# Antibas/eaQHM-analysis-and-synthesis-in-Python

Measured on AMD Instinct MI355X. Metric: analysis_frames_per_sec, higher is better.
Workload: dtype f64; 1 GPU; synth16k_60s_female_maxAdpt5; samples=960000, fs=16000, ls_frames_per_adaptation=63936, adaptations_executed=5, Kmax=59, track_bytes=906240000, parallelism=instants sharded x1 by LS cost; boundary records all-gathered per adaptation

## Files before the change

### eaqhm-analysis-and-synthesis-in-python_amd/csrc/eaqhm_ls_tile.hip

```cpp
#include <type_traits>
#include "eaqhm_ls_common.h"
#include "eaqhm_ls_chol.h"
#include "eaqhm_ls_a0.h"
#include "eaqhm_ls_tilemap.h"
#include "eaqhm_ls_twunits.h"

namespace eaqhm {


#define DIAG_OWNER(jb, nt) ((int)TL_DIAG[nt][jb])
#define TL_THREADS 512
#define TL_WAVES 8
#define TL_CW 8
#define TL_NTMAX 13
#define CI_STRIDE 20
#define CI_NCH 16
#define A0_NS 7
#define A0_M 7

#define TZ_TB 104
#define TZ_NCH 8

__device__ inline void tw_step(d4 (&g)[9], double aR, double aI, double bR, double bI, double nk) {
  const double sA = aR + aI, dB = bI - bR;
  const double naR = nk * aR, naI = nk * aI, nsA = nk * sA;
  const double nbR = nk * bR, nbI = nk * bI, ndB = nk * dB;
  g[0] = __builtin_amdgcn_mfma_f64_16x16x4f64(aR, bR, g[0], 0, 0, 0);
  g[1] = __builtin_amdgcn_mfma_f64_16x16x4f64(aI, bI, g[1], 0, 0, 0);
  g[2] = __builtin_amdgcn_mfma_f64_16x16x4f64(sA, dB, g[2], 0, 0, 0);
  g[3] = __builtin_amdgcn_mfma_f64_16x16x4f64(naR, bR, g[3], 0, 0, 0);
  g[4] = __builtin_amdgcn_mfma_f64_16x16x4f64(naI, bI, g[4], 0, 0, 0);
  g[5] = __builtin_amdgcn_mfma_f64_16x16x4f64(nsA, dB, g[5], 0, 0, 0);
  g[6] = __builtin_amdgcn_mfma_f64_16x16x4f64(naR, nbR, g[6], 0, 0, 0);
  g[7] = __builtin_amdgcn_mfma_f64_16x16x4f64(naI, nbI, g[7], 0, 0, 0);
  g[8] = __builtin_amdgcn_mfma_f64_16x16x4f64(nsA, ndB, g[8], 0, 0, 0);
}

__device__ inline void twu_pair_k3(d4 (&g0)[3], d4 (&g1)[3], d4 (&g2)[3], double aR, double aI, double bR, double bI, double nk) {
  const double sA = aR + aI, dB = bI - bR;
  const double naR = nk * aR, naI = nk * aI, nsA = nk * sA;
  const double nbR = nk * bR, nbI = nk * bI, ndB = nk * dB;
  g0[0] = __builtin_amdgcn_mfma_f64_16x16x4f64(aR, bR, g0[0], 0, 0, 0);
  g0[1] = __builtin_amdgcn_mfma_f64_16x16x4f64(aI, bI, g0[1], 0, 0, 0);
  g0[2] = __builtin_amdgcn_mfma_f64_16x16x4f64(sA, dB, g0[2], 0, 0, 0);
  g1[0] = __builtin_amdgcn_mfma_f64_16x16x4f64(naR, bR, g1[0], 0, 0, 0);
  g1[1] = __builtin_amdgcn_mfma_f64_16x16x4f64(naI, bI, g1[1], 0, 0, 0);
  g1[2] = __builtin_amdgcn_mfma_f64_16x16x4f64(nsA, dB, g1[2], 0, 0, 0);
  g2[0] = __builtin_amdgcn_mfma_f64_16x16x4f64(naR, nbR, g2[0], 0, 0, 0);
  g2[1] = __builtin_amdgcn_mfma_f64_16x16x4f64(naI, nbI, g2[1], 0, 0, 0);
  g2[2] = __builtin_amdgcn_mfma_f64_16x16x4f64(nsA, ndB, g2[2], 0, 0, 0);
}
__device__ inline void twu_pair_2acc(d4 (&g0)[2], d4 (&g1)[2], d4 (&g2)[2], double aR, double aI, double bR, double bI, double nk,
                                     bool k4) {
  const double naR = nk * aR, naI = nk * aI, nbR = nk * bR, nbI = nk * bI;
  g0[0] = __builtin_amdgcn_mfma_f64_16x16x4f64(aR, bR, g0[0], 0, 0, 0);
  g1[0] = __builtin_amdgcn_mfma_f64_16x16x4f64(naR, bR, g1[0], 0, 0, 0);
  g2[0] = __builtin_amdgcn_mfma_f64_16x16x4f64(naR, nbR, g2[0], 0, 0, 0);
  g0[1] = __builtin_amdgcn_mfma_f64_16x16x4f64(aR, bI, g0[1], 0, 0, 0);
  g1[1] = __builtin_amdgcn_mfma_f64_16x16x4f64(naR, bI, g1[1], 0, 0, 0);
  g2[1] = __builtin_amdgcn_mfma_f64_16x16x4f64(naR, nbI, g2[1], 0, 0, 0);
  g0[0] = __builtin_amdgcn_mfma_f64_16x16x4f64(aI, bI, g0[0], 0, 0, 0);
  g1[0] = __builtin_amdgcn_mfma_f64_16x16x4f64(naI, bI, g1[0], 0, 0, 0);
  g2[0] = __builtin_amdgcn_mfma_f64_16x16x4f64(naI, nbI, g2[0], 0, 0, 0);
  if (k4) {
    const double maI = -aI, mnaI = -naI;
    g0[1] = __builtin_amdgcn_mfma_f64_16x16x4f64(maI, bR, g0[1], 0, 0, 0);
    g1[1] = __builtin_amdgcn_mfma_f64_16x16x4f64(mnaI, bR, g1[1], 0, 0, 0);
    g2[1] = __builtin_amdgcn_mfma_f64_16x16x4f64(mnaI, nbR, g2[1], 0, 0, 0);
  }
}

template <int NS, int TW, int UA = 0, int UB = 0>
__device__ __attribute__((noinline)) void tile_frame(const LsArgs& A, int TS_, int ldx_max_, double* lds, int f_) {
  const int TS = uni(TS_), ldx_max = uni(ldx_max_), f = uni(f_);
  const int tid = threadIdx.x, nt_thr = TL_THREADS;
  const int lane = tid & 63;
  const int wave = __builtin_amdgcn_readfirstlane(tid >> 6);
  double* U = uni(lds);
  double* Xre = U;
  double* Xim = Xre + (size_t)TS * ldx_max;
  const size_t usize_g = (size_t)2 * TS * ldx_max;
  double* ci = U + usize_g;
  unsigned long long* masks = (unsigned long long*)(ci + (size_t)CI_STRIDE * 52);
  double* PanR = U;
  double* PanI = PanR + TL_NTMAX * TL_TILE;
  double* WtR = PanI + TL_NTMAX * TL_TILE;
  double* WtI = WtR + TL_NTMAX * TL_TILE;
  double* LdR = WtI + TL_NTMAX * TL_TILE;
  double* LdI = LdR + TL_TILE;
  double* Dc = LdI + TL_TILE;
  double* Zc = Dc + DG_TILE;
  double* zv = Zc + DG_TILE;
  double* xv = zv + 2 * 16 * TL_NTMAX;
  const size_t usize_c = (size_t)(xv + 32 - U);
  double* xs = U + usize_c;
  double* sh = xs + 4 * uni(A.Kcmax);
  double* win = sh + 16;
  double* sig = win + 64 * CI_NCH;
  double* dorig = sig + 64 * CI_NCH;

  const int Npad = ((uni(A.Nmax) + 63) >> 6) << 6;
  double* Qs = uni(A.scratch) + (size_t)blockIdx.x * (size_t)uni((int)A.scratch_stride);
  double* Rs = Qs + (size_t)Npad * uni(A.nmax);
  const bool seeds = uni((int)(A.any_seed && (*A.any_seed != 0))) != 0;
  const double w1 = uni(2.0 * M_PI / A.fs);
  const int PE = TS / 2;
  const double* sA = uni(A.s);
  const int lcol = lane & 15, lq = lane >> 4;
  unsigned long long* dbg = uni(A.debug);
  unsigned long long t_prev = 0;

  {
    const int n = uni(A.ncol[f]);
    const int Kc = 2 * n + 1, Ms = 2 * Kc + 1;
    const int nt = (Ms + 15) >> 4;
    const int c = uni(A.frame_c[f]), wl = uni(A.frame_wl[f]), inst = uni(A.frame_inst[f]);
    const int N = 2 * wl + 1, mid = wl;
    const int T = (Kc + 16) >> 4;
    constexpr int UN = UA + UB;
    constexpr int GA = UA / 3, GB = UB / 3;
    constexpr bool G3 = TW > 0 || UN > 0;
    static_assert(TW == 0 || UN == 0, "whole pairs or units");
    static_assert(UN == 0 || (UA == TWU_UA && UB == TWU_UB), "slot layout of eaqhm_ls_twunits.h");
    const int nb = G3 ? T : nt;
    const int ldx = (nb << 4) + ((nb & 1) ? 0 : 16);
    const int npair = T * (T + 1) / 2;
    const int is = 2 * Kc - 16 * (nt - 1);
    const double f0 = uni(A.f0_stale);
    const int* mycols = uni(A.cols) + (size_t)f * uni(A.Kmax);
    const int npairs = mid + 1;

    if (dbg && tid == 0) t_prev = __builtin_amdgcn_s_memtime();
    for (int q = tid; q < 2 * TS * ldx_max; q += nt_thr) Xre[q] = 0.0;
    for (int t = tid; t < N; t += nt_thr) {
      win[t] = window_value(false, t, N);
      sig[t] = sA[(size_t)(c - wl) + t];
    }
    __syncthreads();
    int* gappy = (int*)(masks + (size_t)52 * CI_NCH);
    prepare_slots<CI_STRIDE, TL_WAVES>(A, Qs, Rs, Npad, ci, masks, gappy, mycols, n, N, mid, c, wl, seeds, lane, wave, CI_NCH);
    LS_STAMP(0);

    constexpr int NM3 = (NS <= 7) ? NS : 0;
    d4 accR[NS], accI[NS], acc3[NM3 ? NM3 : 1];
    int tP[NS], tQ[NS];
    bool live[NS];
#pragma unroll
    for (int sl = 0; sl < NS; ++sl) {
      accR[sl] = (d4){0, 0, 0, 0};
      accI[sl] = (d4){0, 0, 0, 0};
      if (sl < NM3) acc3[sl] = (d4){0, 0, 0, 0};
      const int code = TL_MAP[nt][wave][sl];
      live[sl] = code != 0xFF;
      const int P = live[sl] ? (code >> 4) : 0, Q = live[sl] ? (code & 15) : 0;
      tP[sl] = __builtin_amdgcn_readfirstlane(P);
      tQ[sl] = __builtin_amdgcn_readfirstlane(Q);
    }

    constexpr int TWA = TW ? TW : 1;
    d4 g[TWA][9];
    int gI[TWA], gJ[TWA];
    bool glive[TWA];
#pragma unroll
    for (int sl = 0; sl < TWA; ++sl) {
      const int x = wave + 8 * sl;
      glive[sl] = TW && x < npair;
      int I = 0, J = 0;
      if (glive[sl]) tile_of(x, I, J);
      gI[sl] = __builtin_amdgcn_readfirstlane(I);
      gJ[sl] = __builtin_amdgcn_readfirstlane(J);
#pragma unroll
      for (int p = 0; p < 9; ++p) g[sl][p] = (d4){0, 0, 0, 0};
    }

    constexpr int UAA = UA > 3 ? UA : 3, UBA = UB > 3 ? UB : 3;
    d4 ga[UAA][3], gb[UBA][2];
    int ucode[UN ? UN : 1];
    if constexpr (UN > 0) {
#pragma unroll
      for (int sl = 0; sl < UN; ++sl) ucode[sl] = __builtin_amdgcn_readfirstlane((int)TWU_MAP[wave][sl]);
#pragma unroll
      for (int sl = 0; sl < UA; ++sl)
#pragma unroll
        for (int p = 0; p < 3; ++p) ga[sl][p] = (d4){0, 0, 0, 0};
#pragma unroll
      for (int sl = 0; sl < UB; ++sl) gb[sl][0] = gb[sl][1] = (d4){0, 0, 0, 0};
    }

    for (int d0 = 0; d0 < npairs; d0 += PE) {
#pragma clang loop unroll(disable)
      for (int idx = tid; idx < 16 * n; idx += nt_thr) {
        const int el = idx & 15, j = idx >> 4, d = d0 + el;
        const bool act = d <= mid;
        const int u = mid - d - 1, v = mid + d;
        double su = 0, cu = 1, sv, cv;
        double pur = 0, pui = 0, nur = 0, nui = 0, pvr, pvi, nvr, nvi;
        {
          double* cj = ci + j * CI_STRIDE;
          const double* fb = ((const double**)cj)[2];
          const double* ab = ((const double**)cj)[3];
          const int dc = act ? d : mid;
          const double fu1 = fb[mid - dc], fv = fb[mid + dc];
          const double au = ab[(mid - dc - 1 >= 0) ? (mid - dc - 1) : 0], au1 = ab[mid - dc];
          const double av = ab[mid + dc], av1 = ab[(mid + dc + 1 < N) ? (mid + dc + 1) : (N - 1)];
          const double xu = act ? fu1 : 0.0, xv = (act && d >= 1) ? fv : 0.0;
          const double qv = cj[0] + scan16(xv), qu = -(cj[1] + scan16(xu));
          if (el == 15) { cj[0] = qv; cj[1] = -qu; }
          if (!act) continue;
          const double ainv = cj[17], pr = cj[18], pi = cj[19];
          sincos_cw(qu * w1, &su, &cu);
          sincos_cw(qv * w1, &sv, &cv);
          const double eps = 10e-5;
          if (u >= 0) {
            const double ru = (eps + au) * ainv, rv1 = (eps + av1) * ainv;
            pur = ru * cu;                    pui = ru * su;
            nur = rv1 * (cv * pr - sv * pi);  nui = rv1 * (cv * pi + sv * pr);
          }
          const double rv = (eps + av) * ainv, ru1 = (eps + au1) * ainv;
          pvr = rv * cv;                      pvi = rv * sv;
          nvr = ru1 * (cu * pr - su * pi);    nvi = ru1 * (cu * pi + su * pr);
        }
        double* xr = Xre + (2 * el) * ldx;
        double* xi = Xim + (2 * el) * ldx;
        const int cpos = XCOL(n + 1 + j, el), cneg = XCOL(j, el);
        const int spos = XCOL(Kc + n + 1 + j, el), sneg = XCOL(Kc + j, el);
        const double wv = win[v], nv = (double)(v - mid);
        if (u >= 0) {
          const double wu = win[u], nu = (double)(u - mid);
          pur *= wu; pui *= wu; nur *= wu; nui *= wu;
          xr[cpos] = pur;      xi[cpos] = pui;      xr[cneg] = nur;      xi[cneg] = nui;
          if (!G3) { xr[spos] = nu * pur; xi[spos] = nu * pui; xr[sneg] = nu * nur; xi[sneg] = nu * nui; }
        }
        pvr *= wv; pvi *= wv; nvr *= wv; nvi *= wv;
        xr += ldx; xi += ldx;
        xr[cpos] = pvr;      xi[cpos] = pvi;      xr[cneg] = nvr;      xi[cneg] = nvi;
        if (!G3) { xr[spos] = nv * pvr; xi[spos] = nv * pvi; xr[sneg] = nv * nvr; xi[sneg] = nv * nvi; }
      }
      if ((tid & 15) == 0 && (tid >> 4) < TS) {
        const int row = tid >> 4;
        const int d = d0 + (row >> 1);
        const int t = (row & 1) ? (mid + d) : (mid - d - 1);
        const bool ok = (d <= mid) && (t >= 0);
        const double w = ok ? win[t] : 0.0;
        const double sval = ok ? sig[t] : 0.0;
        const double nn = (double)(t - mid);
        const int el = row >> 1;
        double* xr = Xre + row * ldx;
        double* xi = Xim + row * ldx;
        xr[XCOL(n, el)] = w;               xi[XCOL(n, el)] = 0.0;
        if (!G3) {
          xr[XCOL(Kc + n, el)] = w * nn;   xi[XCOL(Kc + n, el)] = 0.0;
        }
        const int scol = G3 ? Kc : 2 * Kc;
        xr[XCOL(scol, el)] = w * sval;     xi[XCOL(scol, el)] = 0.0;
      }
      if (d0 + PE > mid) {
        for (int q = tid; q < TS * 16 * nb; q += nt_thr) {
          const int row = q / (16 * nb), col = q - row * (16 * nb);
          const int d = d0 + (row >> 1);
          const int t = (row & 1) ? (mid + d) : (mid - d - 1);
          if (d > mid || t < 0) { Xre[row * ldx + col] = 0.0; Xim[row * ldx + col] = 0.0; }
        }
      }
      LS_STAMP(12);
      __syncthreads();
      LS_STAMP(1);
      const int pcs = (npairs - d0 < PE) ? (npairs - d0) : PE;
      const int ksl = (pcs + 1) >> 1;
      if constexpr (UN > 0) {
        const int plane = TS * ldx_max;
        const int kn = (ksl < 8) ? ksl : 8;
#pragma unroll
        for (int gi = 0; gi < GA + GB; ++gi) {
          const int s0 = (gi < GA) ? 3 * gi : UA + 3 * (gi - GA);
          const int code = ucode[s0];
          if (code == 0xFFFF) continue;
          const int ca = 16 * (code >> 8), cb = 16 * ((code >> 4) & 15);
          const bool k4 = (code & 3) == 1;
          int rb = lq * ldx;
          const int sw0 = lcol + (lq >> 1);
          int nk = (lq & 1) ? d0 + (lq >> 1) : -d0 - (lq >> 1) - 1;
          asm volatile("" : "+v"(rb), "+v"(nk));
#pragma clang loop unroll(disable)
          for (int ks = 0; ks < kn; ++ks) {
            const int sw = (sw0 + 2 * ks) & 15;
            const double aR = Xre[rb + ca + sw], aI = Xre[rb + ca + sw + plane];
            const double bR = Xre[rb + cb + sw], bI = Xre[rb + cb + sw + plane];
            rb += 4 * ldx;
            if (gi < GA) {
              const int q = (gi < GA) ? 3 * gi : 0;
              twu_pair_k3(ga[q], ga[q + 1], ga[q + 2], aR, aI, bR, bI, (double)nk);
            } else {
              const int q = (gi >= GA) ? 3 * (gi - GA) : 0;
              twu_pair_2acc(gb[q], gb[q + 1], gb[q + 2], aR, aI, bR, bI, (double)nk, k4);
            }
            nk += (lq & 1) ? 2 : -2;
          }
        }
#pragma unroll
        for (int sl = 0; sl < UN; ++sl) {
          if ((sl < UA) ? (sl < 3 * GA) : (sl - UA < 3 * GB)) continue;
          const int code = ucode[sl];
          if (code == 0xFFFF) continue;
          const int ca = 16 * (code >> 8), cb = 16 * ((code >> 4) & 15), up = (code >> 2) & 3;
          const bool k4 = (code & 3) == 1;
          int rb = lq * ldx;
          const int sw0 = lcol + (lq >> 1);
          int nk = (lq & 1) ? d0 + (lq >> 1) : -d0 - (lq >> 1) - 1;
          asm volatile("" : "+v"(rb), "+v"(nk));
          auto run = [&](auto pc) {
            constexpr int P = decltype(pc)::value;
#pragma clang loop unroll(disable)
            for (int ks = 0; ks < kn; ++ks) {
              const int sw = (sw0 + 2 * ks) & 15;
              double aR = Xre[rb + ca + sw], aI = Xre[rb + ca + sw + plane];
              double bR = Xre[rb + cb + sw], bI = Xre[rb + cb + sw + plane];
              rb += 4 * ldx;
              if constexpr (P >= 1) { aR *= (double)nk; aI *= (double)nk; }
              if constexpr (P == 2) { bR *= (double)nk; bI *= (double)nk; }
              nk += (lq & 1) ? 2 : -2;
              if (sl < UA) {
                d4 (&g)[3] = ga[sl < UA ? sl : 0];
                g[0] = __builtin_amdgcn_mfma_f64_16x16x4f64(aR, bR, g[0], 0, 0, 0);
                g[1] = __builtin_amdgcn_mfma_f64_16x16x4f64(aI, bI, g[1], 0, 0, 0);
                g[2] = __builtin_amdgcn_mfma_f64_16x16x4f64(aR + aI, bI - bR, g[2], 0, 0, 0);
              } else {
                d4 (&g)[2] = gb[sl >= UA ? sl - UA : 0];
                g[0] = __builtin_amdgcn_mfma_f64_16x16x4f64(aR, bR, g[0], 0, 0, 0);
                g[1] = __builtin_amdgcn_mfma_f64_16x16x4f64(aR, bI, g[1], 0, 0, 0);
                g[0] = __builtin_amdgcn_mfma_f64_16x16x4f64(aI, bI, g[0], 0, 0, 0);
                if (k4) g[1] = __builtin_amdgcn_mfma_f64_16x16x4f64(-aI, bR, g[1], 0, 0, 0);
              }
            }
          };
          if (up == 0) run(std::integral_constant<int, 0>{});
          else if (up == 1) run(std::integral_constant<int, 1>{});
          else run(std::integral_constant<int, 2>{});
        }
      } else if constexpr (TW > 0) {
#pragma unroll
        for (int sl = 0; sl < TW; ++sl) {
          if (!glive[sl]) continue;
          const int ca = 16 * gI[sl], cb = 16 * gJ[sl];
          int rb = lq * ldx;
          const int sw0 = lcol + (lq >> 1);
          int nk = (lq & 1) ? d0 + (lq >> 1) : -d0 - (lq >> 1) - 1;
          asm volatile("" : "+v"(rb), "+v"(nk));
          const int plane = TS * ldx_max;
          const int kn = (ksl < 8) ? ksl : 8;
#pragma clang loop unroll(disable)
          for (int ks = 0; ks < kn; ++ks) {
            const int sw = (sw0 + 2 * ks) & 15;
            const double aR = Xre[rb + ca + sw], aI = Xre[rb + ca + sw + plane];
            const double bR = Xre[rb + cb + sw], bI = Xre[rb + cb + sw + plane];
            rb += 4 * ldx;
            tw_step(g[sl], aR, aI, bR, bI, (double)nk);
            nk += (lq & 1) ? 2 : -2;
          }
        }
      } else {
#pragma unroll
        for (int sl = 0; sl < NS; ++sl) {
          if (!live[sl]) continue;
          const int ca = 16 * tP[sl], cb = 16 * tQ[sl];
          int rb = lq * ldx;
          const int sw0 = lcol + (lq >> 1);
          asm volatile("" : "+v"(rb));
          const int plane = TS * ldx_max;
          if (ksl < 8) {
#pragma clang loop unroll(disable)
            for (int ks = 0; ks < ksl; ++ks) {
              const int sw = (sw0 + 2 * ks) & 15;
              const double aR = Xre[rb + ca + sw], aI = Xre[rb + ca + sw + plane];
              const double bR = Xre[rb + cb + sw], bI = Xre[rb + cb + sw + plane];
              rb += 4 * ldx;
              if (sl < NM3) {
                accR[sl] = __builtin_amdgcn_mfma_f64_16x16x4f64(aR, bR, accR[sl], 0, 0, 0);
                acc3[sl < NM3 ? sl : 0] = __builtin_amdgcn_mfma_f64_16x16x4f64(aI, bI, acc3[sl < NM3 ? sl : 0], 0, 0, 0);
                accI[sl] = __builtin_amdgcn_mfma_f64_16x16x4f64(aR + aI, bI - bR, accI[sl], 0, 0, 0);
              } else {
                accR[sl] = __builtin_amdgcn_mfma_f64_16x16x4f64(aR, bR, accR[sl], 0, 0, 0);
                accI[sl] = __builtin_amdgcn_mfma_f64_16x16x4f64(aR, bI, accI[sl], 0, 0, 0);
                accR[sl] = __builtin_amdgcn_mfma_f64_16x16x4f64(aI, bI, accR[sl], 0, 0, 0);
                accI[sl] = __builtin_amdgcn_mfma_f64_16x16x4f64(-aI, bR, accI[sl], 0, 0, 0);
              }
            }
            continue;
          }
          double aR, aI, bR, bI;
          {
            const int sw = sw0 & 15;
            aR = Xre[rb + ca + sw]; aI = Xre[rb + ca + sw + plane]; bR = Xre[rb + cb + sw]; bI = Xre[rb + cb + sw + plane];
          }
#pragma unroll
          for (int ks = 0; ks < 8; ++ks) {
            double naR = 0, naI = 0, nbR = 0, nbI = 0;
            if (ks < 7) {
              rb += 4 * ldx;
              const int sw = (sw0 + 2 * (ks + 1)) & 15;
              naR = Xre[rb + ca + sw]; naI = Xre[rb + ca + sw + plane]; nbR = Xre[rb + cb + sw]; nbI = Xre[rb + cb + sw + plane];
            }
            __builtin_amdgcn_sched_barrier(0);
            if (sl < NM3) {
              accR[sl] = __builtin_amdgcn_mfma_f64_16x16x4f64(aR, bR, accR[sl], 0, 0, 0);
              acc3[sl < NM3 ? sl : 0] = __builtin_amdgcn_mfma_f64_16x16x4f64(aI, bI, acc3[sl < NM3 ? sl : 0], 0, 0, 0);
              accI[sl] = __builtin_amdgcn_mfma_f64_16x16x4f64(aR + aI, bI - bR, accI[sl], 0, 0, 0);
            } else {
              accR[sl] = __builtin_amdgcn_mfma_f64_16x16x4f64(aR, bR, accR[sl], 0, 0, 0);
              accI[sl] = __builtin_amdgcn_mfma_f64_16x16x4f64(aR, bI, accI[sl], 0, 0, 0);
              accR[sl] = __builtin_amdgcn_mfma_f64_16x16x4f64(aI, bI, accR[sl], 0, 0, 0);
              accI[sl] = __builtin_amdgcn_mfma_f64_16x16x4f64(-aI, bR, accI[sl], 0, 0, 0);
            }
            aR = naR; aI = naI; bR = nbR; bI = nbI;
          }
        }
      }
      __syncthreads();
      LS_STAMP(2);
    }
    if constexpr (TW == 0 && NM3 > 0) {
#pragma unroll
      for (int sl = 0; sl < NM3; ++sl) {
        const d4 p1 = accR[sl], p2 = acc3[sl];
        accR[sl] = p1 + p2;
        accI[sl] = accI[sl] + (p1 - p2);
      }
    }
    if constexpr (G3) {
      double* Gs = Qs;
      if constexpr (UN > 0) {
#pragma unroll
        for (int sl = 0; sl < UN; ++sl) {
          const int code = ucode[sl];
          if (code == 0xFFFF) continue;
          const int I = code >> 8, J = (code >> 4) & 15, up = (code >> 2) & 3;
          d4 re, im;
          if (sl < UA) {
            const d4 p1 = ga[sl < UA ? sl : 0][0], p2 = ga[sl < UA ? sl : 0][1];
            re = p1 + p2; im = ga[sl < UA ? sl : 0][2] + (p1 - p2);
          } else {
            re = gb[sl >= UA ? sl - UA : 0][0]; im = gb[sl >= UA ? sl - UA : 0][1];
          }
          double* gt = Gs + (size_t)(up * npair + I * (I + 1) / 2 + J) * 512;
#pragma unroll
          for (int r = 0; r < 4; ++r) {
            const int o = 2 * (16 * (lq + 4 * r) + lcol);
            gt[o] = re[r]; gt[o + 1] = im[r];
          }
        }
      } else
#pragma unroll
      for (int sl = 0; sl < TWA; ++sl) {
        if (!glive[sl]) continue;
        const int x = wave + 8 * sl;
#pragma unroll
        for (int p = 0; p < 3; ++p) {
          const d4 p1 = g[sl][3 * p], p2 = g[sl][3 * p + 1];
          const d4 re = p1 + p2, im = g[sl][3 * p + 2] + (p1 - p2);
          double* gt = Gs + (size_t)(p * npair + x) * 512;
#pragma unroll
          for (int r = 0; r < 4; ++r) {
            const int o = 2 * (16 * (lq + 4 * r) + lcol);
            gt[o] = re[r]; gt[o + 1] = im[r];
          }
        }
      }
      __syncthreads();
#pragma unroll
      for (int sl = 0; sl < NS; ++sl) {
#pragma unroll
        for (int r = 0; r < 4; ++r) {
          const int R = 16 * tP[sl] + lq + 4 * r, C = 16 * tQ[sl] + lcol;
          const bool pad = !live[sl] || R > 2 * Kc || C > 2 * Kc;
          const bool rs = R >= Kc && R < 2 * Kc, cs = C >= Kc && C < 2 * Kc;
          const int a = (R == 2 * Kc) ? Kc : rs ? R - Kc : R, b = (C == 2 * Kc) ? Kc : cs ? C - Kc : C;
          const int p = (int)rs + (int)cs;
          const bool lo = (a >> 4) >= (b >> 4);
          const int I = lo ? (a >> 4) : (b >> 4), J = lo ? (b >> 4) : (a >> 4);
          const int i = lo ? (a & 15) : (b & 15), j = lo ? (b & 15) : (a & 15);
          double vr = 0.0, vi = 0.0;
          if (!pad) {
            const double* gt = Gs + (size_t)(p * npair + I * (I + 1) / 2 + J) * 512;
            const double2 v = *(const double2*)(gt + 2 * (16 * i + j));
            vr = v.x; vi = lo ? v.y : -v.y;
            if (UN > 0 && I == J) vi = v.y - gt[2 * (16 * j + i) + 1];
          }
          accR[sl][r] = vr; accI[sl][r] = vi;
        }
      }
      LS_STAMP(2);
    }

    {
#pragma unroll
      for (int sl = 0; sl < NS; ++sl) {
        if (!live[sl] || tP[sl] != nt - 1) continue;
#pragma unroll
        for (int r = 0; r < 4; ++r) {
          const int row = lq + 4 * r, col = lcol;
          const bool pad = (row > is) || (tQ[sl] == nt - 1 && col > is);
          if (pad) {
            accR[sl][r] = (tQ[sl] == nt - 1 && row == col) ? 1.0 : 0.0;
            accI[sl][r] = 0.0;
          }
        }
      }
#pragma unroll
      for (int sl = 0; sl < NS; ++sl) {
        if (!live[sl] || tP[sl] != tQ[sl]) continue;
#pragma unroll
        for (int r = 0; r < 4; ++r)
          if (lq + 4 * r == lcol) dorig[16 * tP[sl] + lcol] = accR[sl][r];
      }
      double* post = Dc;
      double* dumpD = Dc + DGP_DOUBLES;
      double* zs = dumpD + 128;
      int* dflag = (int*)(zs + 256);
      if (tid == 0) *dflag = 0;
      __syncthreads();
#define TRAILING_UPDATE(sl)                                                                         \
  {                                                                                                 \
    const double* ar = PanR + tP[sl] * TL_TILE;                                                     \
    const double* ai = PanI + tP[sl] * TL_TILE;                                                     \
    const double* br = PanR + tQ[sl] * TL_TILE;                                                     \
    const double* bi = PanI + tQ[sl] * TL_TILE;                                                     \
       \
       \
    d4 p1 = (d4){0, 0, 0, 0}, p2 = (d4){0, 0, 0, 0};                                                \
    _Pragma("unroll") for (int ks = 0; ks < 4; ++ks) {                                              \
      const int o = (4 * ks + lq) * TL_LD + lcol;                                                   \
      const double aR = ar[o], aI = ai[o], lR = br[o], lI = bi[o];                                  \
      p1 = __builtin_amdgcn_mfma_f64_16x16x4f64(aR, lR, p1, 0, 0, 0);                               \
      p2 = __builtin_amdgcn_mfma_f64_16x16x4f64(aI, lI, p2, 0, 0, 0);                               \
      accI[sl] = __builtin_amdgcn_mfma_f64_16x16x4f64(aR + aI, lI - lR, accI[sl], 0, 0, 0);         \
    }                                                                                               \
    accR[sl] = accR[sl] - (p1 + p2);                                                                \
    accI[sl] = accI[sl] + (p1 - p2);                                                                \
  }
      for (int jb = 0; jb < nt; ++jb) {
        d4 Rt = (d4){0, 0, 0, 0}, It = (d4){0, 0, 0, 0};
        bool mine = false;
#pragma unroll
        for (int sl = 0; sl < NS; ++sl) {
          if (!live[sl] || tP[sl] != jb || tQ[sl] != jb) continue;
          if (jb > 0) TRAILING_UPDATE(sl)
          Rt = accR[sl]; It = accI[sl];
          mine = true;
        }
        if (mine) {
          unsigned long long td0 = 0;
          unsigned long long* tlast = (unsigned long long*)(dflag + 2);
          const bool tdiag = dbg && uni(A.debug_diag);
          if (tdiag) td0 = __builtin_amdgcn_s_memtime();
          diag_D(Rt, It, post, nullptr, dflag, 16 * jb, dumpD, LdR, LdI, jb == nt - 1);
          if (tdiag && lane == 0) {
            const unsigned long long td1 = __builtin_amdgcn_s_memtime();
            atomicAdd(dbg + 9, td1 - td0);
            if (jb > 0) { atomicAdd(dbg + 11, td0 - *tlast); atomicAdd(dbg + 14, 1ull); }
            atomicAdd(dbg + 13, 1ull);
            *tlast = td1;
          }
        }
        LS_STAMP(10);
        if (jb > 0) {
#pragma unroll
          for (int sl = 0; sl < NS; ++sl) {
            if (!live[sl] || tQ[sl] < jb || (tP[sl] == jb && tQ[sl] == jb)) continue;
            TRAILING_UPDATE(sl)
          }
        }
        LS_STAMP(8);
        if (!mine && wave == (int)TL_HELP[nt][jb])
          diag_Z(post, dflag, 16 * jb, zs, WtR + jb * TL_TILE, WtI + jb * TL_TILE, dorig + 16 * jb,
                 (jb == nt - 1) ? is : 16, uni(A.fault));
        __syncthreads();
        LS_STAMP(6);
#pragma unroll
        for (int sl = 0; sl < NS; ++sl) {
          if (!live[sl] || tQ[sl] != jb || tP[sl] == jb) continue;
          double* tr = PanR + tP[sl] * TL_TILE;
          double* ti = PanI + tP[sl] * TL_TILE;
#pragma unroll
          for (int r = 0; r < 4; ++r) {
            tr[lcol * TL_LD + lq + 4 * r] = accR[sl][r];
            ti[lcol * TL_LD + lq + 4 * r] = accI[sl][r];
          }
          __builtin_amdgcn_wave_barrier();
          d4 p1 = (d4){0, 0, 0, 0}, p2 = (d4){0, 0, 0, 0}, p3 = (d4){0, 0, 0, 0};
          const double* wr = WtR + jb * TL_TILE;
          const double* wi = WtI + jb * TL_TILE;
#pragma unroll
          for (int ks = 0; ks < 4; ++ks) {
            const int o = (4 * ks + lq) * TL_LD + lcol;
            const double aR = tr[o], aI = ti[o], bR = wr[o], bI = wi[o];
            p1 = __builtin_amdgcn_mfma_f64_16x16x4f64(aR, bR, p1, 0, 0, 0);
            p2 = __builtin_amdgcn_mfma_f64_16x16x4f64(aI, bI, p2, 0, 0, 0);
            p3 = __builtin_amdgcn_mfma_f64_16x16x4f64(aR + aI, bR + bI, p3, 0, 0, 0);
          }
          const d4 xr = p1 - p2, xi = p3 - (p1 + p2);
          accR[sl] = xr; accI[sl] = xi;
          __builtin_amdgcn_wave_barrier();
#pragma unroll
          for (int r = 0; r < 4; ++r) {
            tr[lcol * TL_LD + lq + 4 * r] = xr[r];
            ti[lcol * TL_LD + lq + 4 * r] = xi[r];
          }
        }
        LS_STAMP(7);
        __syncthreads();
      }
#undef TRAILING_UPDATE
      __syncthreads();
      LS_STAMP(3);

#pragma unroll
      for (int sl = 0; sl < NS; ++sl) {
        if (!live[sl] || tP[sl] != nt - 1 || tQ[sl] == nt - 1) continue;
        if (lq == (is & 3)) {
#pragma unroll
          for (int r = 0; r < 4; ++r)
            if (r == (is >> 2)) {
              zv[2 * (16 * tQ[sl] + lcol)] = accR[sl][r];
              zv[2 * (16 * tQ[sl] + lcol) + 1] = -accI[sl][r];
            }
        }
      }
      if (tid < 16) {
        const bool ok = tid < is;
        zv[2 * (16 * (nt - 1) + tid)] = ok ? LdR[is * TL_LD + tid] : 0.0;
        zv[2 * (16 * (nt - 1) + tid) + 1] = ok ? -LdI[is * TL_LD + tid] : 0.0;
      }
      for (int q = tid; q < 4 * Kc; q += nt_thr) xs[q] = 0.0;
      __syncthreads();
      for (int P = nt - 1; P >= 0; --P) {
        if (tid < 256) {
          const int i = tid >> 4, k = tid & 15;
          double xr = 0, xi = 0;
          if (k >= i) {
            const double wr = WtR[P * TL_TILE + i * TL_LD + k], wi = WtI[P * TL_TILE + i * TL_LD + k];
            const double zr = zv[2 * (16 * P + k)], zi = zv[2 * (16 * P + k) + 1];
            xr = wr * zr - wi * zi;
            xi = wr * zi + wi * zr;
          }
#pragma unroll
          for (int o = 8; o > 0; o >>= 1) { xr += __shfl_xor(xr, o); xi += __shfl_xor(xi, o); }
          if (k == 0) {
            xv[2 * i] = xr; xv[2 * i + 1] = xi;
            const int q = 16 * P + i;
            if (q < 2 * Kc) { xs[2 * q] = xr; xs[2 * q + 1] = xi; }
          }
        }
        __syncthreads();
#pragma unroll
        for (int sl = 0; sl < NS; ++sl) {
          if (!live[sl] || tP[sl] != P || tQ[sl] == P) continue;
          double sr = 0, si = 0;
#pragma unroll
          for (int r = 0; r < 4; ++r) {
            const double xr = xv[2 * (lq + 4 * r)], xi = xv[2 * (lq + 4 * r) + 1];
            const double lr = accR[sl][r], li = accI[sl][r];
            sr += lr * xr + li * xi;
            si += lr * xi - li * xr;
          }
          sr += __shfl_xor(sr, 16); si += __shfl_xor(si, 16);
          sr += __shfl_xor(sr, 32); si += __shfl_xor(si, 32);
          if (lq == 0) {
            zv[2 * (16 * tQ[sl] + lcol)] -= sr;
            zv[2 * (16 * tQ[sl] + lcol) + 1] -= si;
          }
        }
        __syncthreads();
      }
      LS_STAMP(4);
    }

    write_record(A, xs, sh, mycols, f, n, inst, c, f0, seeds);
    LS_STAMP(5);
  }
}

__device__ inline int frame_class(int n) {
  const int nt = (2 * (2 * n + 1) + 1 + 15) >> 4;
  return nt <= 8 ? 0 : nt == 9 ? 1 : nt == 10 ? 2 : nt == 11 ? 3 : nt == 12 ? 4 : nt <= TL_NTMAX ? 5 : LS_BIG_CLASS;
}
extern "C" __global__ void __launch_bounds__(256) eaqhm_ls_classify_kernel(LsArgs A) {
  const int f = blockIdx.x * blockDim.x + threadIdx.x, lane = threadIdx.x & 63;
  int cl = (f < A.n_frames) ? frame_class((A.mode == 0) ? A.frame_K[f] : A.ncol[f]) : -1;
  if (f < A.n_frames) {
    if (!frame_window_ok(A, A.frame_c[f], A.frame_wl[f])) { cl = -1; atomicAdd(A.fault + 2, 1); }
  }
  if (A.mode == 1 && cl >= 0) {
    const long long c = A.frame_c[f], wl = A.frame_wl[f];
    const long long lo = (c - wl - 1 > 0) ? (c - wl - 1) : 0;
    for (long long ch = lo >> 10; ch <= ((c + wl) >> 10); ++ch) A.zflag[ch] = 1;
  }
  for (int c = 0; c < LS_NCLS; ++c) {
    const unsigned long long m = __ballot(cl == c);
    if (m == 0ull) continue;
    int base = 0;
    if (lane == __ffsll((long long)m) - 1) base = atomicAdd(A.cls + c, __popcll(m));
    base = __shfl(base, __ffsll((long long)m) - 1);
    if (cl == c) A.cls[16 + (size_t)c * A.n_frames + base + __popcll(m & ((1ull << lane) - 1ull))] = f;
  }
}

extern "C" __global__ void __launch_bounds__(256) eaqhm_ls_zero_prefix_kernel(const double* __restrict__ fm, long long Lt,
                                                                              long long t_lo, int ch0, int zchunks,
                                                                              const unsigned char* __restrict__ zflag,
                                                                              unsigned short* __restrict__ zloc,
                                                                              int* __restrict__ ztot) {
  __shared__ int wsum[4];
  const int k = blockIdx.y, ch = ch0 + blockIdx.x, tid = threadIdx.x, lane = tid & 63, wave = tid >> 6;
  if (!zflag[ch]) return;
  const long long base = (long long)ch << 10;
  int run = 0;
  for (int p = 0; p < 4; ++p) {
    const long long t = base + 256 * p + tid;
    const bool in = t >= t_lo && t < t_lo + Lt;
    const bool z = in && (fm[(size_t)k * Lt + t] == 0.0);
    const unsigned long long m = __ballot(z);
    const int incl = __popcll(m & ((lane == 63) ? ~0ull : ((1ull << (lane + 1)) - 1ull)));
    if (lane == 0) wsum[wave] = __popcll(m);
    __syncthreads();
    int off = 0, tot = 0;
#pragma unroll
    for (int w = 0; w < 4; ++w) { const int v = wsum[w]; tot += v; if (w < wave) off += v; }
    if (in) zloc[(size_t)k * Lt + t] = (unsigned short)(run + off + incl);
    run += tot;
    __syncthreads();
  }
  if (tid == 0) ztot[(size_t)k * zchunks + ch] = run;
}

extern "C" __global__ void __launch_bounds__(TL_THREADS) eaqhm_ls_tile_kernel(LsArgs A, int TS, int ldx_max) {
  extern __shared__ __attribute__((aligned(16))) double lds[];
  __shared__ int nxt;
#define TW_UNITS 0, TWU_UA, TWU_UB
#define RUN_CLASS(NSV, TWV, C)                                                             \
  for (;;) {                                                                             \
    if (threadIdx.x == 0) nxt = atomicAdd(A.cls + 8 + C, 1);                             \
    __syncthreads();                                                                     \
    const int item = nxt;                                                                \
    __syncthreads();                                                                     \
    if (item >= A.cls[C]) break;                                                         \
    if (A.mode == 0) a0_frame<A0_NS, A0_M, 2>(A, lds, A.cls[16 + (size_t)C * A.n_frames + item], TZ_TB, TZ_NCH, 520, 64 * CI_NCH);                          \
    else tile_frame<NSV, TWV>(A, TS, ldx_max, lds, A.cls[16 + (size_t)C * A.n_frames + item]);          \
  }
  RUN_CLASS(12, 0, 5)
  RUN_CLASS(10, TW_UNITS, 4)
  RUN_CLASS(9, TW_UNITS, 3)
  RUN_CLASS(7, 2, 2)
  RUN_CLASS(6, 2, 1)
  RUN_CLASS(5, 2, 0)
#undef RUN_CLASS
#undef TW_UNITS
}

#define TL_LDS_LIMIT (159 * 1024)
static size_t tl_usize_c() {
  return (size_t)4 * TL_NTMAX * TL_TILE + 2 * TL_TILE + 2 * DG_TILE + 2 * 16 * TL_NTMAX + 32;
}
static size_t tl_usize_g(int TS, int ldx_max) { return (size_t)2 * TS * ldx_max + (size_t)CI_STRIDE * 52 + 52 * CI_NCH + 32; }
static size_t tl_lds_doubles(int Kcmax, int TS, int ldx_max) {
  const size_t c = tl_usize_c(), g = tl_usize_g(TS, ldx_max);
  return (c > g ? c : g) + 4 * (size_t)Kcmax + 16 + 2 * 64 * CI_NCH + 16 * TL_NTMAX;
}

bool ls_tile_applicable(int Kcmax, int Nmax) {
  return Nmax <= 64 * CI_NCH && tl_lds_doubles(Kcmax, 32, 16 * TL_NTMAX + 16) * sizeof(double) <= TL_LDS_LIMIT;
}

size_t ls_tile_scratch_stride(int nmax, int Nmax) {
  const size_t Npad = (size_t)((Nmax + 63) >> 6) << 6;
  const size_t bridged = 2 * Npad * nmax, gram = (size_t)3 * 21 * 512;
  return ((bridged > gram ? bridged : gram) + 15) & ~(size_t)15;
}

int launch_ls_prepass(eaqhm_ctx* ctx, LsArgs A, long long track_t0) {
  hipLaunchKernelGGL(eaqhm_ls_classify_kernel, dim3((A.n_frames + 255) / 256), dim3(256), 0, ctx->stream, A);
  HIP_TRY(ctx, hipGetLastError());
  if (A.mode == 1) {
    const int ch0 = (int)(track_t0 >> 10), ch1 = (int)((track_t0 + A.Lt - 1) >> 10);
    hipLaunchKernelGGL(eaqhm_ls_zero_prefix_kernel, dim3(ch1 - ch0 + 1, A.Kmax), dim3(256), 0, ctx->stream, A.fm_cur, A.Lt,
                       track_t0, ch0, A.zchunks, A.zflag, (unsigned short*)A.zloc, (int*)A.ztot);
    HIP_TRY(ctx, hipGetLastError());
  }
  return EAQHM_OK;
}

int launch_ls_tile(eaqhm_ctx* ctx, LsArgs A, int grid) {
  const int Kcmax = A.Kcmax;
  const int ldx_max = 16 * TL_NTMAX + 16;
  const int TS = 32;
  const size_t lds_bytes = tl_lds_doubles(Kcmax, TS, ldx_max) * sizeof(double);
  if (lds_bytes > TL_LDS_LIMIT) return ctx->fail(EAQHM_EINVAL, "eaqhm_ls_batch: LDS budget exceeded (tile variant)");
  if (a0_lds_doubles(A0_M, 2, TZ_TB, TZ_NCH, 520, 64 * CI_NCH, Kcmax) * sizeof(double) > lds_bytes)
    return ctx->fail(EAQHM_EINVAL, "eaqhm_ls_batch: LDS budget exceeded (adaptation 0, tile variant)");
  HIP_TRY(ctx, hipFuncSetAttribute((const void*)eaqhm_ls_tile_kernel, hipFuncAttributeMaxDynamicSharedMemorySize, (int)lds_bytes));
  hipLaunchKernelGGL(eaqhm_ls_tile_kernel, dim3(grid), dim3(TL_THREADS), lds_bytes, ctx->stream, A, TS, ldx_max);
  HIP_TRY(ctx, hipGetLastError());
  return EAQHM_OK;
}

}
```

### eaqhm-analysis-and-synthesis-in-python_amd/csrc/eaqhm_ls_twunits.h

```cpp
#pragma once
namespace eaqhm {
#define TWU_T 6
#define TWU_ACC 20
#define TWU_UA 4
#define TWU_UB 4
__device__ constexpr unsigned short TWU_MAP[8][TWU_UA + TWU_UB] = {
  {0x0400, 0x0404, 0x0408, 0x0524, 0x0421, 0x0425, 0x0429, 0x0549},
  {0x0410, 0x0414, 0x0418, 0x0500, 0x0431, 0x0435, 0x0439, 0xFFFF},
  {0x0100, 0x0104, 0x0108, 0x0504, 0x0002, 0x0006, 0x000A, 0x0529},
  {0x0200, 0x0204, 0x0208, 0x0508, 0x0112, 0x0116, 0x011A, 0x0531},
  {0x0210, 0x0214, 0x0218, 0x0514, 0x0442, 0x0446, 0x044A, 0x0535},
  {0x0300, 0x0304, 0x0308, 0x0510, 0x0552, 0x0556, 0x055A, 0x0539},
  {0x0310, 0x0314, 0x0318, 0x0518, 0x0222, 0x0226, 0x022A, 0x0541},
  {0x0320, 0x0324, 0x0328, 0x0520, 0x0332, 0x0336, 0x033A, 0x0545},
};
constexpr int twu_mfmas(int w) {
  int m = 0;
  for (int s = 0; s < TWU_UA + TWU_UB; ++s)
    if (TWU_MAP[w][s] != 0xFFFF) m += ((TWU_MAP[w][s] & 3) == 1) ? 4 : 3;
  return m;
}
constexpr int twu_count(int I, int J, int p) {
  int c = 0;
  for (int w = 0; w < 8; ++w)
    for (int s = 0; s < TWU_UA + TWU_UB; ++s)
      if (TWU_MAP[w][s] == ((I << 8) | (J << 4) | (p << 2) | (TWU_MAP[w][s] & 3))) ++c;
  return c;
}
constexpr bool twu_every_unit_once() {
  int live = 0;
  for (int w = 0; w < 8; ++w)
    for (int s = 0; s < TWU_UA + TWU_UB; ++s)
      if (TWU_MAP[w][s] != 0xFFFF) ++live;
  if (live != 3 * TWU_T * (TWU_T + 1) / 2) return false;
  for (int I = 0; I < TWU_T; ++I)
    for (int J = 0; J <= I; ++J)
      for (int p = 0; p < 3; ++p)
        if (twu_count(I, J, p) != 1) return false;
  return true;
}
constexpr bool twu_forms_fit_slots() {
  for (int w = 0; w < 8; ++w)
    for (int s = 0; s < TWU_UA + TWU_UB; ++s) {
      const int c = TWU_MAP[w][s];
      if (c == 0xFFFF) continue;
      const int form = c & 3, I = c >> 8, J = (c >> 4) & 15;
      if (form > 2 || (c & 0xC) == 0xC) return false;
      if ((s < TWU_UA) != (form == 0)) return false;
      if ((form == 2) != (I == J)) return false;
    }
  return true;
}
constexpr bool twu_simds_balanced() {
  int lo = 1 << 30, hi = 0;
  for (int w = 0; w < 4; ++w) {
    const int m = twu_mfmas(w) + twu_mfmas(w + 4);
    lo = m < lo ? m : lo;
    hi = m > hi ? m : hi;
  }
  return hi - lo <= 4;
}
constexpr bool twu_pairs_whole() {
  for (int w = 0; w < 8; ++w)
    for (int k = 0; k < 2; ++k) {
      const int s0 = k ? TWU_UA : 0, ng = (k ? TWU_UB : TWU_UA) / 3;
      for (int g = 0; g < ng; ++g) {
        const int c = TWU_MAP[w][s0 + 3 * g];
        for (int p = 0; p < 3; ++p)
          if (TWU_MAP[w][s0 + 3 * g + p] != (c == 0xFFFF ? 0xFFFF : c + (p << 2))) return false;
      }
    }
  return true;
}
static_assert(3 * TWU_UA + 2 * TWU_UB <= TWU_ACC, "accumulator cap per wave");
static_assert(twu_pairs_whole(), "whole pairs in the group slots");
static_assert(twu_every_unit_once(), "every unit (I, J, p) exactly once");
static_assert(twu_forms_fit_slots(), "unit forms against the slot layout");
static_assert(twu_simds_balanced(), "MFMAs per k-step of the four SIMDs equal to within one unit");
}
```

Before: 1.517 million frames/s.

## Pack half-empty edge tile blocks for class-9 frames into fewer MFMA units

```diff
diff --git a/eaqhm-analysis-and-synthesis-in-python_amd/csrc/eaqhm_ls_tile.hip b/eaqhm-analysis-and-synthesis-in-python_amd/csrc/eaqhm_ls_tile.hip
--- a/eaqhm-analysis-and-synthesis-in-python_amd/csrc/eaqhm_ls_tile.hip
+++ b/eaqhm-analysis-and-synthesis-in-python_amd/csrc/eaqhm_ls_tile.hip
@@ -70,7 +70,19 @@
   }
 }
 
-template <int NS, int TW, int UA = 0, int UB = 0>
+__device__ inline void twu_edge_k4(d4 (&g0)[2], d4 (&g1)[2], double aR, double aI, double bR, double bI, double nk) {
+  const double nbR = nk * bR, nbI = nk * bI, maI = -aI;
+  g0[0] = __builtin_amdgcn_mfma_f64_16x16x4f64(aR, bR, g0[0], 0, 0, 0);
+  g1[0] = __builtin_amdgcn_mfma_f64_16x16x4f64(aR, nbR, g1[0], 0, 0, 0);
+  g0[1] = __builtin_amdgcn_mfma_f64_16x16x4f64(aR, bI, g0[1], 0, 0, 0);
+  g1[1] = __builtin_amdgcn_mfma_f64_16x16x4f64(aR, nbI, g1[1], 0, 0, 0);
+  g0[0] = __builtin_amdgcn_mfma_f64_16x16x4f64(aI, bI, g0[0], 0, 0, 0);
+  g1[0] = __builtin_amdgcn_mfma_f64_16x16x4f64(aI, nbI, g1[0], 0, 0, 0);
+  g0[1] = __builtin_amdgcn_mfma_f64_16x16x4f64(maI, bR, g0[1], 0, 0, 0);
+  g1[1] = __builtin_amdgcn_mfma_f64_16x16x4f64(maI, nbR, g1[1], 0, 0, 0);
+}
+
+template <int NS, int TW, int UA = 0, int UB = 0, int TB = 0>
 __device__ __attribute__((noinline)) void tile_frame(const LsArgs& A, int TS_, int ldx_max_, double* lds, int f_) {
   const int TS = uni(TS_), ldx_max = uni(ldx_max_), f = uni(f_);
   const int tid = threadIdx.x, nt_thr = TL_THREADS;
@@ -122,6 +134,9 @@
     constexpr bool G3 = TW > 0 || UN > 0;
     static_assert(TW == 0 || UN == 0, "whole pairs or units");
     static_assert(UN == 0 || (UA == TWU_UA && UB == TWU_UB), "slot layout of eaqhm_ls_twunits.h");
+    static_assert(TB >= 0 && TB < TWU_NTB, "unit table");
+    constexpr bool PK = UN > 0 && TWU_PACKED[TB];
+    constexpr int EC = 16 * (TWU_TT[TB] - 1);
     const int nb = G3 ? T : nt;
     const int ldx = (nb << 4) + ((nb & 1) ? 0 : 16);
     const int npair = T * (T + 1) / 2;
@@ -178,7 +193,7 @@
     int ucode[UN ? UN : 1];
     if constexpr (UN > 0) {
 #pragma unroll
-      for (int sl = 0; sl < UN; ++sl) ucode[sl] = __builtin_amdgcn_readfirstlane((int)TWU_MAP[wave][sl]);
+      for (int sl = 0; sl < UN; ++sl) ucode[sl] = __builtin_amdgcn_readfirstlane((int)TWU_MAPS[TB][wave][sl]);
 #pragma unroll
       for (int sl = 0; sl < UA; ++sl)
 #pragma unroll
@@ -230,11 +245,13 @@
           pur *= wu; pui *= wu; nur *= wu; nui *= wu;
           xr[cpos] = pur;      xi[cpos] = pui;      xr[cneg] = nur;      xi[cneg] = nui;
           if (!G3) { xr[spos] = nu * pur; xi[spos] = nu * pui; xr[sneg] = nu * nur; xi[sneg] = nu * nui; }
+          if (PK && n + 1 + j >= EC) { xr[XCOL(n + 9 + j, el)] = nu * pur; xi[XCOL(n + 9 + j, el)] = nu * pui; }
         }
         pvr *= wv; pvi *= wv; nvr *= wv; nvi *= wv;
         xr += ldx; xi += ldx;
         xr[cpos] = pvr;      xi[cpos] = pvi;      xr[cneg] = nvr;      xi[cneg] = nvi;
         if (!G3) { xr[spos] = nv * pvr; xi[spos] = nv * pvi; xr[sneg] = nv * nvr; xi[sneg] = nv * nvi; }
+        if (PK && n + 1 + j >= EC) { xr[XCOL(n + 9 + j, el)] = nv * pvr; xi[XCOL(n + 9 + j, el)] = nv * pvi; }
       }
       if ((tid & 15) == 0 && (tid >> 4) < TS) {
         const int row = tid >> 4;
@@ -253,6 +270,7 @@
         }
         const int scol = G3 ? Kc : 2 * Kc;
         xr[XCOL(scol, el)] = w * sval;     xi[XCOL(scol, el)] = 0.0;
+        if (PK) { xr[XCOL(Kc + 8, el)] = w * sval * nn;  xi[XCOL(Kc + 8, el)] = 0.0; }
       }
       if (d0 + PE > mid) {
         for (int q = tid; q < TS * 16 * nb; q += nt_thr) {
@@ -275,12 +293,27 @@
           const int s0 = (gi < GA) ? 3 * gi : UA + 3 * (gi - GA);
           const int code = ucode[s0];
           if (code == 0xFFFF) continue;
-          const int ca = 16 * (code >> 8), cb = 16 * ((code >> 4) & 15);
+          const int ca = 16 * ((code >> 8) & 15), cb = 16 * ((code >> 4) & 15);
           const bool k4 = (code & 3) == 1;
           int rb = lq * ldx;
           const int sw0 = lcol + (lq >> 1);
           int nk = (lq & 1) ? d0 + (lq >> 1) : -d0 - (lq >> 1) - 1;
           asm volatile("" : "+v"(rb), "+v"(nk));
+          if (PK && gi >= GA) {
+            if (code & 0x1000) {
+              const int q = (gi >= GA) ? 3 * (gi - GA) : 0;
+#pragma clang loop unroll(disable)
+              for (int ks = 0; ks < kn; ++ks) {
+                const int sw = (sw0 + 2 * ks) & 15;
+                const double aR = Xre[rb + ca + sw], aI = Xre[rb + ca + sw + plane];
+                const double bR = Xre[rb + cb + sw], bI = Xre[rb + cb + sw + plane];
+                rb += 4 * ldx;
+                twu_edge_k4(gb[q], gb[q + 1], aR, aI, bR, bI, (double)nk);
+                nk += (lq & 1) ? 2 : -2;
+              }
+              continue;
+            }
+          }
 #pragma clang loop unroll(disable)
           for (int ks = 0; ks < kn; ++ks) {
             const int sw = (sw0 + 2 * ks) & 15;
@@ -302,7 +335,7 @@
           if ((sl < UA) ? (sl < 3 * GA) : (sl - UA < 3 * GB)) continue;
           const int code = ucode[sl];
           if (code == 0xFFFF) continue;
-          const int ca = 16 * (code >> 8), cb = 16 * ((code >> 4) & 15), up = (code >> 2) & 3;
+          const int ca = 16 * ((code >> 8) & 15), cb = 16 * ((code >> 4) & 15), up = (code >> 2) & 3;
           const bool k4 = (code & 3) == 1;
           int rb = lq * ldx;
           const int sw0 = lcol + (lq >> 1);
@@ -316,8 +349,8 @@
               double aR = Xre[rb + ca + sw], aI = Xre[rb + ca + sw + plane];
               double bR = Xre[rb + cb + sw], bI = Xre[rb + cb + sw + plane];
               rb += 4 * ldx;
-              if constexpr (P >= 1) { aR *= (double)nk; aI *= (double)nk; }
-              if constexpr (P == 2) { bR *= (double)nk; bI *= (double)nk; }
+              if constexpr (P == 1 || P == 2) { aR *= (double)nk; aI *= (double)nk; }
+              if constexpr (P >= 2) { bR *= (double)nk; bI *= (double)nk; }
               nk += (lq & 1) ? 2 : -2;
               if (sl < UA) {
                 d4 (&g)[3] = ga[sl < UA ? sl : 0];
@@ -334,6 +367,7 @@
             }
           };
           if (up == 0) run(std::integral_constant<int, 0>{});
+          else if (PK && (code & 0x1000)) run(std::integral_constant<int, PK ? 3 : 1>{});
           else if (up == 1) run(std::integral_constant<int, 1>{});
           else run(std::integral_constant<int, 2>{});
         }
@@ -433,7 +467,7 @@
         for (int sl = 0; sl < UN; ++sl) {
           const int code = ucode[sl];
           if (code == 0xFFFF) continue;
-          const int I = code >> 8, J = (code >> 4) & 15, up = (code >> 2) & 3;
+          const int I = (code >> 8) & 15, J = (code >> 4) & 15, up = (code >> 2) & 3;
           d4 re, im;
           if (sl < UA) {
             const d4 p1 = ga[sl < UA ? sl : 0][0], p2 = ga[sl < UA ? sl : 0][1];
@@ -480,10 +514,14 @@
           const int i = lo ? (a & 15) : (b & 15), j = lo ? (b & 15) : (a & 15);
           double vr = 0.0, vi = 0.0;
           if (!pad) {
-            const double* gt = Gs + (size_t)(p * npair + I * (I + 1) / 2 + J) * 512;
-            const double2 v = *(const double2*)(gt + 2 * (16 * i + j));
+            const bool edge = PK && I == T - 1;
+            const int q = (edge && I != J) ? (int)(p == 2) : edge ? 0 : p;
+            const int ii = edge ? i + ((I != J) ? 8 * (p - q) : (p >= 1 ? 8 : 0)) : i;
+            const int jj = (edge && I == J && p == 2) ? j + 8 : j;
+            const double* gt = Gs + (size_t)(q * npair + I * (I + 1) / 2 + J) * 512;
+            const double2 v = *(const double2*)(gt + 2 * (16 * ii + jj));
             vr = v.x; vi = lo ? v.y : -v.y;
-            if (UN > 0 && I == J) vi = v.y - gt[2 * (16 * j + i) + 1];
+            if (UN > 0 && I == J) vi = v.y - gt[2 * (16 * jj + ii) + 1];
           }
           accR[sl][r] = vr; accI[sl][r] = vi;
         }
@@ -735,7 +773,7 @@
 extern "C" __global__ void __launch_bounds__(TL_THREADS) eaqhm_ls_tile_kernel(LsArgs A, int TS, int ldx_max) {
   extern __shared__ __attribute__((aligned(16))) double lds[];
   __shared__ int nxt;
-#define TW_UNITS 0, TWU_UA, TWU_UB
+#define TW_UNITS(TB) 0, TWU_UA, TWU_UB, TB
 #define RUN_CLASS(NSV, TWV, C)                                                             \
   for (;;) {                                                                             \
     if (threadIdx.x == 0) nxt = atomicAdd(A.cls + 8 + C, 1);                             \
@@ -747,8 +785,8 @@
     else tile_frame<NSV, TWV>(A, TS, ldx_max, lds, A.cls[16 + (size_t)C * A.n_frames + item]);          \
   }
   RUN_CLASS(12, 0, 5)
-  RUN_CLASS(10, TW_UNITS, 4)
-  RUN_CLASS(9, TW_UNITS, 3)
+  RUN_CLASS(10, TW_UNITS(TWU_TB_12), 4)
+  RUN_CLASS(9, TW_UNITS(TWU_TB_11), 3)
   RUN_CLASS(7, 2, 2)
   RUN_CLASS(6, 2, 1)
   RUN_CLASS(5, 2, 0)
diff --git a/eaqhm-analysis-and-synthesis-in-python_amd/csrc/eaqhm_ls_twunits.h b/eaqhm-analysis-and-synthesis-in-python_amd/csrc/eaqhm_ls_twunits.h
--- a/eaqhm-analysis-and-synthesis-in-python_amd/csrc/eaqhm_ls_twunits.h
+++ b/eaqhm-analysis-and-synthesis-in-python_amd/csrc/eaqhm_ls_twunits.h
@@ -1,80 +1,110 @@
 #pragma once
 namespace eaqhm {
-#define TWU_T 6
 #define TWU_ACC 20
 #define TWU_UA 4
 #define TWU_UB 4
-__device__ constexpr unsigned short TWU_MAP[8][TWU_UA + TWU_UB] = {
-  {0x0400, 0x0404, 0x0408, 0x0524, 0x0421, 0x0425, 0x0429, 0x0549},
-  {0x0410, 0x0414, 0x0418, 0x0500, 0x0431, 0x0435, 0x0439, 0xFFFF},
-  {0x0100, 0x0104, 0x0108, 0x0504, 0x0002, 0x0006, 0x000A, 0x0529},
-  {0x0200, 0x0204, 0x0208, 0x0508, 0x0112, 0x0116, 0x011A, 0x0531},
-  {0x0210, 0x0214, 0x0218, 0x0514, 0x0442, 0x0446, 0x044A, 0x0535},
-  {0x0300, 0x0304, 0x0308, 0x0510, 0x0552, 0x0556, 0x055A, 0x0539},
-  {0x0310, 0x0314, 0x0318, 0x0518, 0x0222, 0x0226, 0x022A, 0x0541},
-  {0x0320, 0x0324, 0x0328, 0x0520, 0x0332, 0x0336, 0x033A, 0x0545},
+#define TWU_NTB 2
+#define TWU_TB_12 0
+#define TWU_TB_11 1
+__device__ constexpr int TWU_TT[TWU_NTB] = {6, 6};
+__device__ constexpr bool TWU_PACKED[TWU_NTB] = {false, true};
+__device__ constexpr unsigned short TWU_MAPS[TWU_NTB][8][TWU_UA + TWU_UB] = {
+  {
+    {0x0400, 0x0404, 0x0408, 0x0524, 0x0421, 0x0425, 0x0429, 0x0549},
+    {0x0410, 0x0414, 0x0418, 0x0500, 0x0431, 0x0435, 0x0439, 0xFFFF},
+    {0x0100, 0x0104, 0x0108, 0x0504, 0x0002, 0x0006, 0x000A, 0x0529},
+    {0x0200, 0x0204, 0x0208, 0x0508, 0x0112, 0x0116, 0x011A, 0x0531},
+    {0x0210, 0x0214, 0x0218, 0x0514, 0x0442, 0x0446, 0x044A, 0x0535},
+    {0x0300, 0x0304, 0x0308, 0x0510, 0x0552, 0x0556, 0x055A, 0x0539},
+    {0x0310, 0x0314, 0x0318, 0x0518, 0x0222, 0x0226, 0x022A, 0x0541},
+    {0x0320, 0x0324, 0x0328, 0x0520, 0x0332, 0x0336, 0x033A, 0x0545},
+  },
+  {
+    {0x0400, 0x0404, 0x0408, 0x1544, 0x0421, 0x0425, 0x0429, 0xFFFF},
+    {0x0410, 0x0414, 0x0418, 0x1540, 0x0431, 0x0435, 0x0439, 0xFFFF},
+    {0x0100, 0x0104, 0x0108, 0x1510, 0x0002, 0x0006, 0x000A, 0x1552},
+    {0x0200, 0x0204, 0x0208, 0x1514, 0x0112, 0x0116, 0x011A, 0xFFFF},
+    {0x0310, 0x0314, 0x0318, 0x1524, 0x0442, 0x0446, 0x044A, 0xFFFF},
+    {0x0320, 0x0324, 0x0328, 0x1520, 0x1501, 0x1505, 0xFFFF, 0xFFFF},
+    {0x0210, 0x0214, 0x0218, 0x1530, 0x0222, 0x0226, 0x022A, 0xFFFF},
+    {0x0300, 0x0304, 0x0308, 0x1534, 0x0332, 0x0336, 0x033A, 0xFFFF},
+  },
 };
-constexpr int twu_mfmas(int w) {
+constexpr int twu_mfmas(int tb, int w) {
   int m = 0;
   for (int s = 0; s < TWU_UA + TWU_UB; ++s)
-    if (TWU_MAP[w][s] != 0xFFFF) m += ((TWU_MAP[w][s] & 3) == 1) ? 4 : 3;
+    if (TWU_MAPS[tb][w][s] != 0xFFFF) m += ((TWU_MAPS[tb][w][s] & 3) == 1) ? 4 : 3;
   return m;
 }
-constexpr int twu_count(int I, int J, int p) {
+constexpr int twu_count(int tb, int key) {
   int c = 0;
   for (int w = 0; w < 8; ++w)
     for (int s = 0; s < TWU_UA + TWU_UB; ++s)
-      if (TWU_MAP[w][s] == ((I << 8) | (J << 4) | (p << 2) | (TWU_MAP[w][s] & 3))) ++c;
+      if (TWU_MAPS[tb][w][s] != 0xFFFF && (TWU_MAPS[tb][w][s] & ~3) == key) ++c;
   return c;
 }
-constexpr bool twu_every_unit_once() {
+constexpr bool twu_every_entry_once(int tb) {
+  const int T = TWU_TT[tb], E = T - 1;
+  const bool pk = TWU_PACKED[tb];
   int live = 0;
   for (int w = 0; w < 8; ++w)
     for (int s = 0; s < TWU_UA + TWU_UB; ++s)
-      if (TWU_MAP[w][s] != 0xFFFF) ++live;
-  if (live != 3 * TWU_T * (TWU_T + 1) / 2) return false;
-  for (int I = 0; I < TWU_T; ++I)
-    for (int J = 0; J <= I; ++J)
-      for (int p = 0; p < 3; ++p)
-        if (twu_count(I, J, p) != 1) return false;
-  return true;
-}
-constexpr bool twu_forms_fit_slots() {
-  for (int w = 0; w < 8; ++w)
-    for (int s = 0; s < TWU_UA + TWU_UB; ++s) {
-      const int c = TWU_MAP[w][s];
-      if (c == 0xFFFF) continue;
-      const int form = c & 3, I = c >> 8, J = (c >> 4) & 15;
-      if (form > 2 || (c & 0xC) == 0xC) return false;
-      if ((s < TWU_UA) != (form == 0)) return false;
-      if ((form == 2) != (I == J)) return false;
+      if (TWU_MAPS[tb][w][s] != 0xFFFF) ++live;
+  if (live != (pk ? 3 * E * (E + 1) / 2 + 2 * E + 1 : 3 * T * (T + 1) / 2)) return false;
+  for (int I = 0; I < T; ++I)
+    for (int J = 0; J <= I; ++J) {
+      const int key = (I << 8) | (J << 4);
+      if (pk && I == E) {
+        if (twu_count(tb, 0x1000 | key) != 1) return false;
+        if (J < E && twu_count(tb, 0x1000 | key | (1 << 2)) != 1) return false;
+      } else {
+        for (int p = 0; p < 3; ++p)
+          if (twu_count(tb, key | (p << 2)) != 1) return false;
+      }
     }
   return true;
 }
-constexpr bool twu_simds_balanced() {
+constexpr bool twu_forms_fit_slots(int tb) {
+  for (int w = 0; w < 8; ++w)
+    for (int s = 0; s < TWU_UA + TWU_UB; ++s) {
+      const int c = TWU_MAPS[tb][w][s];
+      if (c == 0xFFFF) continue;
+      const int form = c & 3, I = (c >> 8) & 15, J = (c >> 4) & 15, p = (c >> 2) & 3;
+      const bool edge = (c & 0x1000) != 0;
+      if ((c & ~0x1FFF) || form > 2 || p == 3 || I >= TWU_TT[tb] || J > I) return false;
+      if ((s < TWU_UA) != (form == 0)) return false;
+      if ((form == 2) != (I == J)) return false;
+      if (edge != (TWU_PACKED[tb] && I == TWU_TT[tb] - 1)) return false;
+      if (edge && p > (I == J ? 0 : 1)) return false;
+    }
+  return true;
+}
+constexpr bool twu_simds_balanced(int tb) {
   int lo = 1 << 30, hi = 0;
   for (int w = 0; w < 4; ++w) {
-    const int m = twu_mfmas(w) + twu_mfmas(w + 4);
+    const int m = twu_mfmas(tb, w) + twu_mfmas(tb, w + 4);
     lo = m < lo ? m : lo;
     hi = m > hi ? m : hi;
   }
   return hi - lo <= 4;
 }
-constexpr bool twu_pairs_whole() {
+constexpr bool twu_pairs_whole(int tb) {
   for (int w = 0; w < 8; ++w)
     for (int k = 0; k < 2; ++k) {
       const int s0 = k ? TWU_UA : 0, ng = (k ? TWU_UB : TWU_UA) / 3;
       for (int g = 0; g < ng; ++g) {
-        const int c = TWU_MAP[w][s0 + 3 * g];
+        const int c = TWU_MAPS[tb][w][s0 + 3 * g];
+        const bool edge = c != 0xFFFF && (c & 0x1000);
+        if (edge && (k == 0 || ((c >> 8) & 15) == ((c >> 4) & 15))) return false;
         for (int p = 0; p < 3; ++p)
-          if (TWU_MAP[w][s0 + 3 * g + p] != (c == 0xFFFF ? 0xFFFF : c + (p << 2))) return false;
+          if (TWU_MAPS[tb][w][s0 + 3 * g + p] != ((c == 0xFFFF || (edge && p == 2)) ? 0xFFFF : c + (p << 2))) return false;
       }
     }
   return true;
 }
 static_assert(3 * TWU_UA + 2 * TWU_UB <= TWU_ACC, "accumulator cap per wave");
-static_assert(twu_pairs_whole(), "whole pairs in the group slots");
-static_assert(twu_every_unit_once(), "every unit (I, J, p) exactly once");
-static_assert(twu_forms_fit_slots(), "unit forms against the slot layout");
-static_assert(twu_simds_balanced(), "MFMAs per k-step of the four SIMDs equal to within one unit");
+static_assert(twu_pairs_whole(TWU_TB_12) && twu_pairs_whole(TWU_TB_11), "whole pairs in the group slots");
+static_assert(twu_every_entry_once(TWU_TB_12) && twu_every_entry_once(TWU_TB_11), "every entry of every G_p from exactly one unit");
+static_assert(twu_forms_fit_slots(TWU_TB_12) && twu_forms_fit_slots(TWU_TB_11), "unit forms against the slot layout");
+static_assert(twu_simds_balanced(TWU_TB_12) && twu_simds_balanced(TWU_TB_11), "MFMAs per k-step of the four SIMDs equal to within one unit");
 }
```

New measurement: 1.548 million frames/s, median of 6. 1.02x the previous value.
